# QCLovers/PyTDSCF

Measured on AMD Instinct MI355X. Metric: tdvp_sweeps_per_sec, higher is better.
Workload: dtype c128; 1 GPU; C4: synthetic exciton chain L=64 d=16 D=1024 M=32; L=64, d=16, D=1024, M=32, integrator=lanczos, steps_per_half_sweep=8, parallelism=single, approximate=False

## Files before the change

### pytdscf_amd/csrc/engine.h

```cpp
#pragma once
#include <functional>
#include <map>
#include <memory>
#include <string>
#include <vector>

#include "../../include/mitdvp.h"
#include "common.h"
#include "krylov_dev.h"
#include "qr.h"
#include "small_site.h"
#include "svd.h"
#include "vecops.h"

namespace mitdvp {

struct DevBuf {
  zc* p = nullptr;
  size_t n = 0;
  DevBuf() = default;
  DevBuf(const DevBuf&) = delete;
  DevBuf& operator=(const DevBuf&) = delete;
  DevBuf(DevBuf&& o) noexcept : p(o.p), n(o.n) { o.p = nullptr; o.n = 0; }
  DevBuf& operator=(DevBuf&& o) noexcept {
    if (this != &o) { release(); p = o.p; n = o.n; o.p = nullptr; o.n = 0; }
    return *this;
  }
  ~DevBuf() { release(); }
  void release() {
    if (p) (void)hipFree(p);
    p = nullptr;
    n = 0;
  }
  void reserve(size_t elems) {
    if (elems <= n) return;
    release();
    if (elems == 0) return;
    HIP_CHECK(hipMalloc(&p, elems * sizeof(zc)));
    n = elems;
  }
  void grow_preserve(size_t elems, size_t used, hipStream_t st) {
    if (elems <= n) return;
    zc* q = nullptr;
    HIP_CHECK(hipMalloc(&q, elems * sizeof(zc)));
    if (p && used) {
      HIP_CHECK(hipMemcpyAsync(q, p, used * sizeof(zc), hipMemcpyDeviceToDevice, st));
      HIP_CHECK(hipStreamSynchronize(st));
    }
    release();
    p = q;
    n = elems;
  }
};

struct ApplyPlan {
  bool trim_l = false, trim_r = false, edge = false, fold_l = false, fold_r = false;
  int strassen_l = 0, strassen_r = 0;
};

struct MpoSite {
  int ml = 0, d = 0, mr = 0;
  DevBuf w2l;
  DevBuf w2r;
  DevBuf w2lt, w2rt, kl_l, kl_r;
  int kl_stride_l = 0, kl_stride_r = 0;
  double sp_frac_l = 1.0, sp_frac_r = 1.0;
  struct SpSeg { int r0, r1; bool dense; int tile0; };
  std::vector<SpSeg> seg_l, seg_r;
  DevBuf w2el;
  DevBuf w2er;
  std::vector<hzc> whost;
  std::vector<char> nzblk;
  struct EnvFold {
    std::vector<int> t0; DevBuf ws, wg; bool reuse = false; hzc reuse_alpha; DevBuf ws_reuse;
    DevBuf ws_list, ws_reuse_list, wg_list; size_t wg_list_stride = 0;
  };
  struct EdgeCache {
    bool valid = false;
    unsigned long long s = 0, e = 0;
    std::vector<hzc> lam, mu;
    bool has_l = false, has_r = false;
    int skip = 0;
    DevBuf w_l, w_r;
    DevBuf w_l_list, w_r_list;
    DevBuf w_lf, w_rf;
    bool lf_ok = false, rf_ok = false;
    EnvFold envf[2];
    void rebuild(hipStream_t st, const MpoSite& w, unsigned long long S, unsigned long long E, const std::vector<hzc>& lam,
                 const std::vector<hzc>& mu);
  };
  mutable EdgeCache edge;
  DevBuf wtr;
  int ntr = 0, mltr = 0, mrtr = 0;
  int dtr = 0;
  bool set = false;
};
struct Operator {
  std::vector<MpoSite> sites;
  hzc shift{0.0, 0.0};
};

typedef int (*CollFn)(void* user, int op, void* dev_ptr, size_t nbytes);
enum { COLL_ALLGATHER = 0, COLL_ALLREDUCE = 1 };

struct PhaseTimer {
  hipEvent_t a, b;
  int kind;
  bool closed;
};

class SiteShard;
class Batch;
void cu_range_claim(int device, int first, int count);
void cu_range_release(int device, int first, int count);
int cu_ranges_claimed(int device);

class Engine {
  friend class SiteShard;
  friend class Batch;
// ... 108 lines not shown
  void copy_out(double* dst, const zc* src, size_t elems);
  void fold_block(int op_id, bool conj_bra, bool from_left, const double* in, int d, int m, double* out, int first = 0,
                  int count = -1);
  void site_rdm_blocks(int isite, const double* TL, const double* TR, double* out);
  hipStream_t stream() const { return st_; }
  int kprev_get(int p);
  void kprev_set(int p, int k);
  void set_small_kernels(bool on);
  void check_device_errors() { ss_check(); }
  const SmallSync::Last& small_last() const { return ss_.last; }
  const MpoSite& mpo(int op_id, int isite);
  mitdvp_config cfg;

 private:
  int ptr_mode_ = 0;
  struct CuClaim {
    int dev = -1, first = 0, count = 0;
    ~CuClaim() { if (dev >= 0) cu_range_release(dev, first, count); }
  } cu_claim_;
  bool qr_gauge_free_ = true;
  bool trim_identity_ = true;
  int edge_mode_ = -1;
  int fold_mode_ = -1;
  int strassen_mode_ = -1;
  bool strassen_batched_ = true;
  bool strassen_fuse_ = true;
  DevBuf str_l_, str_r_, str_v_, str_m_;
  static bool try_reserve(DevBuf& b, size_t elems);
  void strassen_side(const zc* fixed, bool fixed_is_a, const zc* psi, long ldpsi, zc* out, long hm, long hn, long hk, bool accumulate,
                     int level);
  int fold_env_mode_ = -1;
  bool env_reuse_ = true;
  bool core_lists_ = true;
  struct EnvChecked { const MpoSite* w = nullptr; const zc* blk[2] = {nullptr, nullptr}; int n[2] = {0, 0}; int lvl[2] = {0, 0}; } env_chk_;
  EnvChecked take_env_checked() { const EnvChecked c = env_chk_; env_chk_ = EnvChecked{}; return c; }
  struct IdentRecord { double dev[128]; hzc lam[128]; };
  static_assert(sizeof(IdentRecord) == 128 * 8 + 128 * 16 && sizeof(IdentRecord) <= 4 * NPART * sizeof(zc), "layout of the identity-check record");
  const IdentRecord& identity_sets(const zc* L, int ml, int dl, unsigned long long ms, const zc* R, int mr, int dr, unsigned long long me);
  void identity_blocks(const zc* L, int dl, int ml, const zc* R, int dr, int mr, bool* left, bool* right);
  int L_;
  hipStream_t st_ = nullptr;
  std::vector<int> dl_, dd_, dr_, gauge_;
  std::vector<DevBuf> site_;
  std::vector<std::vector<int>> sub_;
  std::vector<int> subn_;
  std::map<int, Operator> ops_;
  int center_ = -1;
  bool segment_ = false;
  int bnd_dl_ = 1, bnd_ml_ = 1, bnd_dr_ = 1, bnd_mr_ = 1;
  int bond_ = -1, bond_dim_ = 0, bond_site_ = 0;

  std::vector<DevBuf> envL_, envR_;
  std::vector<char> envL_ok_, envR_ok_;
  std::vector<DevBuf> pool_;
  size_t pool_cap_ = 48;
  DevBuf pool_get(size_t elems);
  void pool_put(DevBuf&& b);

  DevBuf X_, Y_, V_, Vdiag_, tmp1_, tmp2_, sig_, sig2_, qrwork_, red_;
  int max_diag_krylov_ = 64;
  MappedHost<zc> h_red_;
  MappedHost<unsigned> h_seq_;
  unsigned seq_tag_ = 0;
  KryDev* kst_ = nullptr;
  MappedHost<KryPub> h_kpub_;
  unsigned kry_tag_ = 0;
// ... 98 lines not shown
```

### pytdscf_amd/csrc/engine.hip

```cpp
#include "engine_internal.h"
#include "engine_krylov.inc"
#include "rccl_dyn.h"

namespace mitdvp {

Engine::Engine(const mitdvp_config& c) : cfg(c), L_(c.nsite) {
  if (c.nsite < 1) throw ArgError("nsite must be >= 1");
  if (c.max_krylov < 1 || c.max_krylov > MAXK - 1) throw ArgError("max_krylov must be in [1, 20]");
  if (c.integrator != MITDVP_LANCZOS && c.integrator != MITDVP_ARNOLDI) throw ArgError("bad integrator");
  if (c.relax < 0 || c.relax > 2) throw ArgError("relax must be 0, 1 or 2");
  max_diag_krylov_ = c.max_diag_krylov > 0 ? c.max_diag_krylov : 64;
  if (const char* e = std::getenv("MITDVP_SMALL_KERNELS")) small_kernels_ = std::atoi(e) != 0;
  if (const char* e = std::getenv("MITDVP_SPARSE_W")) sparse_w_ = std::atoi(e) != 0;
  if (const char* e = std::getenv("MITDVP_TRIM_IDENTITY")) trim_identity_ = std::atoi(e) != 0;
  if (const char* e = std::getenv("MITDVP_EDGE_APPLY")) edge_mode_ = std::atoi(e);
  if (const char* e = std::getenv("MITDVP_FOLD_APPLY")) fold_mode_ = std::atoi(e);
  if (const char* e = std::getenv("MITDVP_FOLD_STRASSEN")) strassen_mode_ = std::atoi(e);
  if (const char* e = std::getenv("MITDVP_STRASSEN_BATCH")) strassen_batched_ = std::atoi(e) != 0;
  if (const char* e = std::getenv("MITDVP_STRASSEN_FUSE")) strassen_fuse_ = std::atoi(e) != 0;
  if (const char* e = std::getenv("MITDVP_FOLD_ENV")) fold_env_mode_ = std::atoi(e);
  if (const char* e = std::getenv("MITDVP_FOLD_ENV_REUSE")) env_reuse_ = std::atoi(e) != 0;
  if (const char* e = std::getenv("MITDVP_CORE_LISTS")) core_lists_ = std::atoi(e) != 0;
  if (const char* e = std::getenv("MITDVP_QR_GAUGE_FREE")) qr_gauge_free_ = std::atoi(e) != 0;
  if (const char* e = std::getenv("MITDVP_KEFF_IDENT")) keff_ident_ = std::atoi(e) != 0;
  int ndev = 0;
  HIP_CHECK(hipGetDeviceCount(&ndev));
  if (ndev < 1) throw HipError("no HIP device visible: the MI355X engine has no CPU fallback");
  if (c.device < 0 || c.device >= ndev) throw ArgError("bad device ordinal");
  HIP_CHECK(hipSetDevice(c.device));
  HIP_CHECK(hipDeviceGetAttribute(&n_cu_, hipDeviceAttributeMultiprocessorCount, c.device));
  if (c.cu_count > 0) {
    if (c.cu_first < 0 || c.cu_first + c.cu_count > n_cu_ || c.cu_count % 8 != 0 || c.cu_first % 8 != 0)
      throw ArgError("cu_first / cu_count: a multiple of 8 compute units inside the device (8 k units = k CUs on every XCD)");
    std::vector<uint32_t> mask((size_t)(n_cu_ + 31) / 32, 0u);
    for (int u = c.cu_first; u < c.cu_first + c.cu_count; ++u) mask[(size_t)u / 32] |= 1u << (u % 32);
    cu_range_claim(c.device, c.cu_first, c.cu_count);
    cu_claim_.dev = c.device; cu_claim_.first = c.cu_first; cu_claim_.count = c.cu_count;
    HIP_CHECK(hipExtStreamCreateWithCUMask(&st_, (uint32_t)mask.size(), mask.data()));
    n_cu_ = c.cu_count;
    ss_.max_grid = c.cu_count;
    ss_.partitioned = true;
  } else {
    HIP_CHECK(hipStreamCreate(&st_));
  }
  qr_hist_ = qr_history_new();
  dl_.assign(L_, 0); dd_.assign(L_, 0); dr_.assign(L_, 0); gauge_.assign(L_, -1);
  site_.resize(L_);
  sub_.assign(L_, {}); subn_.assign(L_, 0);
  envL_.resize(L_ + 1); envR_.resize(L_ + 1);
  envL_ok_.assign(L_ + 1, 0); envR_ok_.assign(L_ + 1, 0);
  kprev_.assign(L_, 0);
  red_.reserve(RED_TOTAL);
  red_elems_ = RED_TOTAL;
  h_red_.alloc(RED_TOTAL * sizeof(zc));
  h_seq_.alloc(64);
// ... 702 lines not shown
```

### pytdscf_amd/csrc/engine_apply.hip

```cpp
#include "engine_internal.h"
#include "core_lists.h"

namespace mitdvp {

constexpr long STRASSEN_MIN_TILES = 256;

double Engine::w_stage(const MpoSite* sp, int side, const zc* w2, int d, int mout, int min_, int ncol, int nbatch) {
  ZgemmDesc g = zgemm_desc(w2, X_.p, Y_.p, d * mout, ncol, min_ * d);
  g.batch = nbatch; g.strideA = 0; g.strideB = (long)min_ * d * ncol; g.strideC = (long)d * mout * ncol;
  const bool use = sp && sparse_w_ && ncol >= 64 && (side == 0 ? sp->kl_l.p : sp->kl_r.p) &&
                   (side == 0 ? sp->sp_frac_l : sp->sp_frac_r) <= 0.6;
  if (!use) {
    zgemm(st_, g);
    return 1.0;
  }
  const zc* wt = side == 0 ? sp->w2lt.p : sp->w2rt.p;
  const int* kl = reinterpret_cast<const int*>(side == 0 ? sp->kl_l.p : sp->kl_r.p);
  const int stride = side == 0 ? sp->kl_stride_l : sp->kl_stride_r;
  const auto& segs = side == 0 ? sp->seg_l : sp->seg_r;
  const int K = min_ * d;
  for (int pass = 0; pass < 2; ++pass)
    for (const auto& sgm : segs) {
      if (sgm.dense != (pass == 0)) continue;
      ZgemmDesc h = g;
      h.A = wt + (size_t)sgm.r0 * K;
      h.M = sgm.r1 - sgm.r0;
      h.rowmap_p = d; h.rowmap_s1 = (long)mout * ncol; h.rowmap_s2 = ncol; h.rowmap_r0 = sgm.r0;
      if (!sgm.dense) { h.klist = kl + (size_t)sgm.tile0 * stride; h.klist_stride = stride; }
      h.tile_cfg = (sgm.dense && h.M <= 32) ? 2 : 1;
      zgemm(st_, h);
      cnt_.n_launch += 1;
    }
  cnt_.n_launch -= 1;
  return side == 0 ? sp->sp_frac_l : sp->sp_frac_r;
// ... 213 lines not shown
  if (same) return;
  const hzc* W = w.whost.data();
  std::vector<hzc> wl((size_t)d * ml * d, hzc(0, 0)), wr((size_t)d * d * mr, hzc(0, 0));
  valid = has_l = has_r = false;
  for (int c = 0; c < ml; ++c)
    for (int t = 0; t < mr; ++t) {
      if (!w.nzblk[(size_t)c * mr + t]) continue;
      const bool in_s = (S >> c) & 1ull;
      const hzc f = in_s ? lam[c] : mu[t];
      if (f == hzc(0.0, 0.0)) continue;
      for (int i = 0; i < d; ++i)
        for (int j = 0; j < d; ++j) {
          const hzc v = f * W[(((size_t)c * d + i) * d + j) * mr + t];
          if (in_s) wr[(size_t)i * d * mr + (size_t)j * mr + t] += v;
          else wl[(size_t)i * ml * d + (size_t)c * d + j] += v;
        }
      (in_s ? has_r : has_l) = true;
    }
  w_l.reserve(wl.size());
  w_r.reserve(wr.size());
  HIP_CHECK(hipMemcpyAsync(w_l.p, wl.data(), wl.size() * sizeof(zc), hipMemcpyHostToDevice, st));
  HIP_CHECK(hipMemcpyAsync(w_r.p, wr.data(), wr.size() * sizeof(zc), hipMemcpyHostToDevice, st));
  auto upload_list = [&](DevBuf& b, const std::vector<unsigned char>& blob, size_t at = 0) {
    HIP_CHECK(hipMemcpyAsync(reinterpret_cast<unsigned char*>(b.p) + at, blob.data(), blob.size(), hipMemcpyHostToDevice, st));
    HIP_CHECK(hipStreamSynchronize(st));
  };
  {
    const std::vector<unsigned char> ll = build_fold_list(wl.data(), d, ml, (long)ml * d, 1, d);
    const std::vector<unsigned char> lr = build_fold_list(wr.data(), d, mr, (long)d * mr, mr, 1);
    w_l_list.reserve(ll.size() / sizeof(zc));
    w_r_list.reserve(lr.size() / sizeof(zc));
    upload_list(w_l_list, ll);
    upload_list(w_r_list, lr);
  }
  w_lf.reserve(wl.size());
  w_rf.reserve(wr.size());
  lf_ok = zgemm_reduce_pack_core(st, w_l.p, (long)ml * d, d, ml * d, w_lf.p);
  rf_ok = zgemm_reduce_pack_core(st, w_r.p, (long)d * mr, d, d * mr, w_rf.p);
  for (int side = 0; side < 2; ++side) {
    const int mi = side == 0 ? ml : mr, mo = side == 0 ? mr : ml;
    const unsigned long long I = side == 0 ? S : E;
    const std::vector<hzc>& wt = side == 0 ? lam : mu;
    auto blk = [&](int in, int out) { return side == 0 ? (size_t)in * mr + out : (size_t)out * mr + in; };
    auto Wel = [&](int in, int i, int j, int out) {
      return side == 0 ? W[(((size_t)in * d + i) * d + j) * mr + out] : W[(((size_t)out * d + i) * d + j) * mr + in];
    };
    EnvFold& f = envf[side];
    f.t0.clear();
    for (int out = 0; out < mo; ++out)
      for (int in = 0; in < mi; ++in)
        if (!((I >> in) & 1ull) && w.nzblk[blk(in, out)]) { f.t0.push_back(out); break; }
    std::vector<hzc> ws((size_t)d * d * mo, hzc(0, 0)), wg(std::max<size_t>(f.t0.size(), 1) * d * mi * d, hzc(0, 0));
    for (int in = 0; in < mi; ++in) {
      if (!((I >> in) & 1ull)) continue;
      for (int out = 0; out < mo; ++out) {
        if (!w.nzblk[blk(in, out)]) continue;
        for (int i = 0; i < d; ++i)
          for (int j = 0; j < d; ++j) ws[((size_t)i * d + j) * mo + out] += wt[in] * Wel(in, i, j, out);
      }
    }
    for (size_t k = 0; k < f.t0.size(); ++k)
      for (int in = 0; in < mi; ++in) {
        if (((I >> in) & 1ull) || !w.nzblk[blk(in, f.t0[k])]) continue;
        for (int i = 0; i < d; ++i)
          for (int j = 0; j < d; ++j) wg[((k * d + i) * mi + in) * d + j] = Wel(in, i, j, f.t0[k]);
      }
// ... 56 lines not shown
  const bool skip = edge_cand && w.edge.skip > 0;
  if (skip) w.edge.skip -= 1;
  if (!edge_cand || skip) {
    identity_blocks(trim_identity_ && dl >= 256 && ml > 1 ? Lb : nullptr, dl, ml,
                    trim_identity_ && dr >= 256 && mr > 1 ? Rb : nullptr, dr, mr, &plan.trim_l, &plan.trim_r);
    return plan;
  }
  unsigned long long S = 0, E = 0;
  std::vector<hzc> lam(ml), mu(mr);
  for (int attempt = (w.edge.valid ? 0 : 1); attempt < 2; ++attempt) {
    const unsigned long long ms = attempt == 0 ? w.edge.s : ~0ull, me = attempt == 0 ? w.edge.e : ~0ull;
    const IdentRecord& h = identity_sets(Lb, ml, dl, ms, Rb, mr, dr, me);
    S = E = 0;
    for (int c = 0; c < ml; ++c) { lam[c] = h.lam[c]; if (((ms >> c) & 1ull) && h.dev[c] < 1e-13) S |= 1ull << c; }
    for (int t = 0; t < mr; ++t) { mu[t] = h.lam[64 + t]; if (((me >> t) & 1ull) && h.dev[64 + t] < 1e-13) E |= 1ull << t; }
    if (attempt == 0 && (S != w.edge.s || E != w.edge.e)) continue;
    break;
  }
  plan.trim_l = ml > 1 && (S & 1ull) && std::abs(lam[0] - 1.0) < 1e-13;
  plan.trim_r = mr > 1 && ((E >> (mr - 1)) & 1ull) && std::abs(mu[mr - 1] - 1.0) < 1e-13;
  for (int c = 0; c < ml; ++c)
    for (int t = 0; t < mr; ++t)
      if (w.nzblk[(size_t)c * mr + t] && !((S >> c) & 1ull) && !((E >> t) & 1ull)) {
        w.edge.skip = 16;
        return plan;
      }
  w.edge.rebuild(st_, w, S, E, lam, mu);
  plan.edge = true;
  env_chk_ = EnvChecked{&w, {Lb, Rb}, {dl, dr}};
  plan.fold_r = w.edge.has_r && can_fold_r;
  plan.fold_l = w.edge.has_l && can_fold_l;
  if (plan.fold_r || plan.fold_l) {
    timer_begin(11);
    if (plan.fold_r)
      fold_env_core(st_, Rb, w.edge.w_r.p, Y_.p, dr, mr, d, (long)d * mr, mr, 1, (long)dr * d * dr, (long)d * dr, dr, 1,
                    core_lists_ ? w.edge.w_r_list.p : nullptr);
    if (plan.fold_l)
      fold_env_core(st_, Lb, w.edge.w_l.p, X_.p, dl, ml, d, (long)ml * d, 1, d, (long)dl * d, (long)d * dl * d, 1, d,
                    core_lists_ ? w.edge.w_l_list.p : nullptr);
    const size_t quarter = (size_t)dl * d * dr / 4;
    auto tiles_fill = [](long pm, long pn) { return ((pm + 63) / 64) * ((pn + 63) / 64) >= STRASSEN_MIN_TILES; };
    auto level_of = [&](long rows, long cols, long klen) {
      if (strassen_mode_ == 0 || rows % 2 || cols % 2 || klen % 2) return 0;
      const bool four = rows % 4 == 0 && cols % 4 == 0 && klen % 4 == 0;
      if (strassen_mode_ > 0) return strassen_mode_ >= 2 && four ? 2 : 1;
      if (four && tiles_fill(rows / 4, cols / 4)) return 2;
      return tiles_fill(rows / 2, cols / 2) ? 1 : 0;
    };
    auto pack = [&](const zc* op, long n, DevBuf& f, int which, int want) {
      const long h = n / 2, q = n / 4;
      const size_t two = (strassen_fuse_ && which == STRASSEN_A ? 0 : 7 * quarter) + 49 * (quarter / 4);
      if (want == 2 && try_reserve(f, 49 * (size_t)q * q) && try_reserve(str_v_, two) && try_reserve(str_m_, two)) {
        strassen_operands2(st_, op, n, q, q, f.p, which);
        cnt_.n_launch += 1;
        return 2;
      }
      if (want == 0 || !try_reserve(f, 7 * (size_t)h * h) || !try_reserve(str_v_, 7 * quarter) || !try_reserve(str_m_, 7 * quarter))
        return 0;
      strassen_operands(st_, op, n, h, h, f.p, which);
      cnt_.n_launch += 1;
      return 1;
    };
    if (plan.fold_r) plan.strassen_r = pack(Y_.p, (long)d * dr, str_r_, STRASSEN_BT, level_of(dl, (long)d * dr, (long)d * dr));
    if (plan.fold_l) plan.strassen_l = pack(X_.p, (long)dl * d, str_l_, STRASSEN_A, level_of((long)dl * d, dr, (long)dl * d));
    env_chk_.lvl[0] = plan.strassen_l;
    env_chk_.lvl[1] = plan.strassen_r;
    timer_end();
    cnt_.n_launch += (plan.fold_r ? 1 : 0) + (plan.fold_l ? 1 : 0);
    if (std::getenv("MITDVP_EDGE_TRACE"))
      fprintf(stderr, "[mitdvp] folded sides of a site: R %s, L %s\n",
              plan.strassen_r == 2 ? "49 quarter-size products" : plan.strassen_r ? "seven half-size products" : plan.fold_r ? "plain product" : "not folded",
              plan.strassen_l == 2 ? "49 quarter-size products" : plan.strassen_l ? "seven half-size products" : plan.fold_l ? "plain product" : "not folded");
  }
  return plan;
}

void Engine::heff_apply(const zc* L, const MpoSite& w, const zc* R, const zc* psi, zc* out, int dl, int d, int dr,
                        hzc shift, const ApplyPlan& plan) {
  SmallChain sc;
  if (small_ok() && chain_heff(sc, L, w, R, dl, d, dr, false)) {
    timer_begin(10);
    small_apply(st_, ss_, sc, psi, out, ss_partials(sc), make_double2(shift.real(), shift.imag()), shift != hzc(0.0, 0.0));
    timer_end();
    cnt_.n_launch += 1;
    cnt_.n_heff += 1;
    cnt_.heff_flops += 8.0 * ((double)dl * dl * w.ml * d * dr + (double)dl * dr * w.ml * w.mr * d * d + (double)dl * dr * dr * w.mr * d);
    return;
  }
  if (plan.edge) heff_apply_edge(L, w, R, psi, out, dl, d, dr, plan);
  else heff_apply_rect(L, w, R, psi, out, dl, dl, d, dr, dr, plan);
  if (shift != hzc(0.0, 0.0))
    vec_axpby(st_, out, psi, (long)dl * d * dr, make_double2(shift.real(), shift.imag()), make_double2(1.0, 0.0));
}

void Engine::keff_apply_rect(const zc* L, const zc* R, const zc* sig, zc* out, int dlo, int dli, int dro, int dri,
                             int m) {
  int a0, a1;
  const bool sharded = shard_range(dlo, a0, a1);
  const int na = a1 - a0;
  timer_begin(2);
  {
    ZgemmDesc g = zgemm_desc(L + (size_t)a0 * m * dli, sig, X_.p, na * m, dri, dli);
    zgemm(st_, g);
  }
  {
// ... 219 lines not shown
```

### pytdscf_amd/csrc/engine_segment.hip

```cpp
#include "engine_internal.h"
#include "engine_krylov.inc"

namespace mitdvp {

void Engine::replace_site(int i, const double* reim, int gauge) {
  if (i < 0 || i >= L_ || !site_[i].p) throw ArgError("replace_site: bad or unset site");
  const size_t e = (size_t)dl_[i] * dd_[i] * dr_[i];
  copy_in(site_[i].p, reim, e);
  gauge_[i] = gauge;
  if (gauge == MITDVP_GAUGE_PSI) center_ = i;
  else if (center_ == i) center_ = -1;
}

void Engine::reshape_site(int i, const double* reim, int l, int n, int r, int gauge) {
  if (i < 0 || i >= L_ || !site_[i].p) throw ArgError("reshape_site: bad or unset site");
  if (l < 1 || r < 1 || n != dd_[i]) throw ArgError("reshape_site: bad shape");
  if (i != 0 && i != L_ - 1) throw ArgError("reshape_site: only a block's first or last site faces a junction");
  if ((i > 0 && l != dl_[i]) || (i < L_ - 1 && r != dr_[i])) throw ArgError("reshape_site: only the outer bond may change");
  const size_t e = (size_t)l * n * r;
  site_[i].reserve(e);
  copy_in(site_[i].p, reim, e);
  dl_[i] = l; dr_[i] = r; gauge_[i] = gauge;
  if (gauge == MITDVP_GAUGE_PSI) center_ = i;
  else if (center_ == i) center_ = -1;
// ... 40 lines not shown

void Engine::site_exp(double dt) {
  require_ready();
  if (center_ < 0) throw ArgError("site_exp: no centre site");
  const int p = center_;
  if (!envL_ok_[p] || !envR_ok_[p + 1]) throw ArgError("site_exp: the environment blocks around the centre are not built");
  local_site_exp(p, dt);
  ss_check();
}

void Engine::heff_apply_center(const double* in, double* out, int* flags) {
  require_ready();
  if (center_ < 0) throw ArgError("heff_apply_center: no centre site");
  const int p = center_;
  if (!envL_ok_[p] || !envR_ok_[p + 1]) throw ArgError("heff_apply_center: the environment blocks around the centre are not built");
  const MpoSite& w = mpo(0, p);
  if (dd_[p] != w.d) throw ArgError("MPO physical dimension differs from the site tensor's");
  const int dl = dl_[p], d = dd_[p], dr = dr_[p];
  const size_t n = (size_t)dl * d * dr;
  const zc* Lb = envL_[p].p;
  const zc* Rb = envR_[p + 1].p;
  DevBuf x = pool_get(n), y = pool_get(n);
  if (in) copy_in(x.p, in, n);
  else HIP_CHECK(hipMemcpyAsync(x.p, site_[p].p, n * sizeof(zc), hipMemcpyDeviceToDevice, st_));
  const ApplyPlan plan = choose_apply_forms(Lb, w, Rb, dl, d, dr);
  SmallChain sc;
  const bool small = small_ok() && chain_heff(sc, Lb, w, Rb, dl, d, dr, false);
  const bool edge = plan.edge && !small;
  const bool sparse = !small && !edge && sparse_w_ && dr >= 64 && w.kl_l.p && w.sp_frac_l <= 0.6;
  if (flags)
    *flags = (plan.trim_l && !small && !edge ? 1 : 0) | (plan.trim_r && !small && !edge ? 2 : 0) | (sparse ? 4 : 0) | (small ? 8 : 0) |
             (edge ? 16 : 0) | (edge && plan.fold_r ? 0x20 : 0) | (edge && plan.fold_l ? 0x40 : 0) |
             (edge && plan.strassen_r ? 0x80 : 0) | (edge && plan.strassen_l ? 0x100 : 0) |
             (edge && plan.strassen_r == 2 ? 0x200 : 0) | (edge && plan.strassen_l == 2 ? 0x400 : 0);
  heff_apply(Lb, w, Rb, x.p, y.p, dl, d, dr, op(0).shift, plan);
  copy_out(out, y.p, n);
  pool_put(std::move(x)); pool_put(std::move(y));
}

void Engine::split_center(bool forward) {
  require_ready();
  if (center_ < 0) throw ArgError("split_center: no centre site");
  const int p = center_;
  const MpoSite& w = mpo(0, p);
  const int dl = dl_[p], d = dd_[p], dr = dr_[p];
  DevBuf spare = pool_get(V_.n / MAXK);
  if (forward) {
    if (!envL_ok_[p]) throw ArgError("split_center: left environment missing");
    timer_begin(3);
    long nl = 0;
    qr_thin(st_, site_[p].p, dl * d, dr, spare.p, sig_.p, qrwork_.p, &nl, qr_hist_, qr_gauge_free_);
    timer_end();
    cnt_.n_launch += nl; cnt_.n_qr += 1;
    std::swap(site_[p], spare);
    gauge_[p] = MITDVP_GAUGE_A;
    pool_put(std::move(envL_[p + 1]));
    envL_[p + 1] = pool_get((size_t)dr * w.mr * dr);
    env_update(envL_[p].p, site_[p].p, w.w2l.p, envL_[p + 1].p, dl, w.ml, d, dr, w.mr, w.w2el.p, &w, 0);
    envL_ok_[p + 1] = 1;
    bond_ = p + 1; bond_dim_ = dr;
  } else {
    if (!envR_ok_[p + 1]) throw ArgError("split_center: right environment missing");
    gauge_qr_right(site_[p].p, dl, d, dr, spare.p, tmp2_.p, sig_.p);
    std::swap(site_[p], spare);
    gauge_[p] = MITDVP_GAUGE_B;
    pool_put(std::move(envR_[p]));
    envR_[p] = pool_get((size_t)dl * w.ml * dl);
// ... 171 lines not shown
```

### pytdscf_amd/csrc/vecops.h

```cpp
#pragma once
#include "common.h"
#include "small_chain_plan.h"

namespace mitdvp {

constexpr int NPART = 256;

constexpr int SMALL_VEC_EPT = 16;
constexpr long SMALL_VEC_N = 1024L * SMALL_VEC_EPT;

struct Coefs {
  zc c[MAXK];
};

int vec_blocks(long n);
void vec_dot(hipStream_t st, const zc* x, const zc* y, long n, bool conj_x, zc* out_p );
void vec_sumsq(hipStream_t st, const zc* x, long n, double* out_p );
void vec_lanczos_update(hipStream_t st, zc* v, const zc* vm1, const zc* vm2 , long n,
                        const zc* alpha_p, const double* betaprev_p, double* out_p);
void vec_lanczos_update_deferred(hipStream_t st, zc* v, const zc* ul, const zc* ulm1 , long n, const zc* alpha_raw_p,
                                 const double* nrm_all, int l, bool orthodox, double eps, double* out_p);
void vec_lanczos_step_small(hipStream_t st, zc* w, const zc* x, const zc* vl, const zc* vm2 , long n,
                            zc* alpha_p, const double* betaprev_p, double* nrm_p, double eps);
void vec_scale_inv_norm(hipStream_t st, zc* v, long n, const double* nrm_p, double eps);
void vec_multi_dot(hipStream_t st, const zc* V, long ldv, int k, const zc* v, long n, zc* out_p );
void vec_arnoldi_update(hipStream_t st, zc* v, const zc* V, long ldv, int k, long n, const zc* h_p, double* out_p);
void vec_lincomb(hipStream_t st, zc* out , const zc* V, long ldv, int k, const Coefs& c, long n,
                 double* nrm_p );
void vec_axpby(hipStream_t st, zc* y, const zc* x, long n, zc a, zc b);
void vec_scale(hipStream_t st, zc* y, long n, zc a);
void vec_randn(hipStream_t st, zc* out, long n, uint64_t seed);
void set_identity(hipStream_t st, zc* out, int rows, int cols, long ld);
void vec_copy_raw(hipStream_t st, zc* dst, const zc* src, size_t n);
void ident_deviation(hipStream_t st, const zc* blk, long ld, int n, double* out_dev);
void ident_deviation_multi(hipStream_t st, const zc* base, int nblk, long blk_stride, long ld, int n, double* out_dev,
                           zc* lam_dev, unsigned long long mask = ~0ull, bool clear = true);
void fold_env_core(hipStream_t st, const zc* env, const zc* w, zc* G, int n, int m, int d, long wi, long wj, long wm, long gi,
                   long gp, long gj, long gq, const void* list = nullptr);
void gram_env_core(hipStream_t st, const zc* G, const zc* ws, zc* out, int n, int m, int d, const void* list = nullptr);
void gram_mirror_lower(hipStream_t st, zc* G, int n, int d);
enum { STRASSEN_A = 0, STRASSEN_B = 1, STRASSEN_BT = 2 };
void strassen_operands(hipStream_t st, const zc* src, long ld, long hr, long hc, zc* dst, int which, int batch = 1,
                       long sstride = 0, long dstride = 0);
void strassen_operands2(hipStream_t st, const zc* src, long ld, long qr, long qc, zc* dst, int which);
void strassen_combine(hipStream_t st, const zc* M, long hr, long hc, zc* out, long ldo, bool accumulate, int batch = 1,
                      long mstride = 0, long ostride = 0);
void strassen_combine2(hipStream_t st, const zc* M, long qr, long qc, zc* out, long ldo, bool accumulate);
void copy2d(hipStream_t st, zc* dst, long ldd, const zc* src, long lds, long rows, int cols, int zero_to, zc a,
            bool accumulate);
struct BlockList { int n; int idx[64]; zc f[64]; };
void gather_blocks(hipStream_t st, zc* dst, int n_dst, const zc* src, int m_src, long rows, int cols, const BlockList& bl);
void fill_scaled_blocks(hipStream_t st, zc* X, long ldx, int pos0, const zc* sig, long rows, int cols, const BlockList& bl);
void accum_scaled_blocks(hipStream_t st, zc* out, const zc* X, long ldx, const zc* sig, long rows, int cols, const BlockList& bl,
                         zc both);
void col_sumsq(hipStream_t st, const zc* x, long rows, int cols, double* out );
void row_sumsq(hipStream_t st, const zc* x, int rows, long cols, double* out );
void shell_sumsq(hipStream_t st, const zc* x, int n, double* out );
void transpose_batched(hipStream_t st, const zc* in, zc* out, int rows, int cols, long ldi, long ldo, int batch,
                       long in_bs, long out_bs);
void phys_diag(hipStream_t st, const zc* C, zc* out, int dl, int n, int dr, bool trace);
void permute_0213(hipStream_t st, const zc* in, zc* out, long n0, int n1, int n2, int n3);
void clock_probe(hipStream_t st, long iters, double* host_out3 );
void where_probe(const uint32_t* mask, int nwords, int nblocks, size_t lds_bytes, int spin_us, int* host_out);
void permute5(hipStream_t st, const zc* in, zc* out, const int dims[5], const long in_strides[5], const int* map2);
void scale_cols(hipStream_t st, zc* x, long rows, int cols, long ld, const double* sc_dev);
void transpose_rev3(hipStream_t st, const zc* in, zc* out, int na, int nj, int ns);

}
```

### pytdscf_amd/csrc/vecops.hip

```cpp
#include "vecops.h"
#include "core_lists.h"
#include "krylov_dev.h"

#include <algorithm>

namespace mitdvp {

__device__ __forceinline__ double wave_sum(double v) {
#pragma unroll
  for (int o = 32; o > 0; o >>= 1) v += __shfl_down(v, o, 64);
  return v;
}

__device__ __forceinline__ double block_sum(double v, double* sh ) {
  v = wave_sum(v);
  const int lane = threadIdx.x & 63, w = threadIdx.x >> 6;
  __syncthreads();
  if (lane == 0) sh[w] = v;
  __syncthreads();
  if (threadIdx.x == 0) sh[4] = sh[0] + sh[1] + sh[2] + sh[3];
  __syncthreads();
  return sh[4];
}

__device__ __forceinline__ zc sum_partials_z(const zc* p, int np, double* sh) {
  double re = 0, im = 0;
  for (int i = threadIdx.x; i < np; i += 256) { re += p[i].x; im += p[i].y; }
  re = block_sum(re, sh);
  im = block_sum(im, sh);
  return make_double2(re, im);
}
__device__ __forceinline__ double sum_partials_d(const double* p, int np, double* sh) {
  double re = 0;
  for (int i = threadIdx.x; i < np; i += 256) re += p[i];
// ... 990 lines not shown
    }
  }
}
__global__ __launch_bounds__(256) void k_gram_mirror_lower(zc* G, int n, int d) {
  __shared__ zc tile[32][33];
  int i = 1, j = blockIdx.z;
  while (j >= i) { j -= i; ++i; }
  const long ldg = (long)d * n;
  const int q0 = blockIdx.x * 32, p0 = blockIdx.y * 32;
  const int tx = threadIdx.x & 31, ty = threadIdx.x >> 5;
  const zc* src = G + ((long)j * n) * ldg + (long)i * n;
  zc* dst = G + ((long)i * n) * ldg + (long)j * n;
  for (int r = ty; r < 32; r += 8) {
    const int q = q0 + r, p = p0 + tx;
    if (q < n && p < n) tile[r][tx] = src[(long)q * ldg + p];
  }
  __syncthreads();
  for (int r = ty; r < 32; r += 8) {
    const int p = p0 + r, q = q0 + tx;
    if (p < n && q < n) {
      const zc v = tile[tx][r];
      dst[(long)p * ldg + q] = make_double2(v.x, -v.y);
    }
  }
}
void gram_mirror_lower(hipStream_t st, zc* G, int n, int d) {
  if (n < 1 || d < 2) return;
  if (n > 65535 || d > 64) throw ArgError("gram_mirror_lower: d <= 64 and bond dimension <= 65535");
  const int nt = (n + 31) / 32;
  hipLaunchKernelGGL(k_gram_mirror_lower, dim3(nt, nt, d * (d - 1) / 2), dim3(256), 0, st, G, n, d);
  HIP_CHECK(hipGetLastError());
}

struct StrassenTab { int q1[7], q2[7], sg[7]; };
constexpr StrassenTab kStrassenTabs[3] = {
    {{0, 2, 0, 3, 0, 2, 1}, {3, 3, 0, 0, 1, 0, 3}, {1, 1, 0, 0, 1, -1, -1}},
    {{0, 0, 1, 2, 3, 0, 2}, {3, 0, 3, 0, 0, 1, 3}, {1, 0, -1, -1, 0, 1, 1}},
    {{0, 0, 2, 1, 3, 0, 1}, {3, 0, 3, 0, 0, 2, 3}, {1, 0, -1, -1, 0, 1, 1}}};
template <int W>
__global__ __launch_bounds__(256) void k_strassen_operands(const zc* __restrict__ src, long ld, long hr, long hc,
                                                           zc* __restrict__ dst, long sstride, long dstride) {
  constexpr StrassenTab t = kStrassenTabs[W];
  const long c = (long)blockIdx.x * 256 + threadIdx.x;
  if (c >= hc) return;
  const long blk = hr * hc;
  src += blockIdx.z * sstride;
  dst += blockIdx.z * dstride;
  for (long r = blockIdx.y; r < hr; r += gridDim.y) {
    zc q[4];
    q[0] = src[r * ld + c];
    q[1] = src[r * ld + hc + c];
    q[2] = src[(hr + r) * ld + c];
    q[3] = src[(hr + r) * ld + hc + c];
#pragma unroll
    for (int k = 0; k < 7; ++k) {
      const zc a = q[t.q1[k]], b = q[t.q2[k]];
      zc o = a;
      if (t.sg[k] > 0) { o.x += b.x; o.y += b.y; }
      if (t.sg[k] < 0) { o.x -= b.x; o.y -= b.y; }
      dst[k * blk + r * hc + c] = o;
    }
  }
}
template <int W>
__global__ __launch_bounds__(256) void k_strassen_operands2(const zc* __restrict__ src, long ld, long qr, long qc,
                                                            zc* __restrict__ dst) {
  constexpr StrassenTab t = kStrassenTabs[W];
  const long c = (long)blockIdx.x * 256 + threadIdx.x;
  if (c >= qc) return;
  const long blk = qr * qc;
  for (long r = blockIdx.y; r < qr; r += gridDim.y) {
// ... 151 lines not shown
```

Measured before the change: 0.04565 sweeps/s.

## Build Strassen operand factors directly from environment and MPO core in one MFMA kernel

New measurement: 0.04597 sweeps/s (median of 6 runs). Within noise of the previous version (+0.7%).

```diff
diff --git a/pytdscf_amd/csrc/engine.h b/pytdscf_amd/csrc/engine.h
--- a/pytdscf_amd/csrc/engine.h
+++ b/pytdscf_amd/csrc/engine.h
@@ -56,6 +56,7 @@
 struct ApplyPlan {
   bool trim_l = false, trim_r = false, edge = false, fold_l = false, fold_r = false;
   int strassen_l = 0, strassen_r = 0;
+  bool direct_l = false, direct_r = false;
 };
 
 struct MpoSite {
@@ -83,8 +84,10 @@
     int skip = 0;
     DevBuf w_l, w_r;
     DevBuf w_l_list, w_r_list;
+    DevBuf w_rd[2];
     DevBuf w_lf, w_rf;
     bool lf_ok = false, rf_ok = false;
+    bool rd_ok[2] = {false, false};
     EnvFold envf[2];
     void rebuild(hipStream_t st, const MpoSite& w, unsigned long long S, unsigned long long E, const std::vector<hzc>& lam,
                  const std::vector<hzc>& mu);
@@ -259,6 +262,7 @@
   int fold_env_mode_ = -1;
   bool env_reuse_ = true;
   bool core_lists_ = true;
+  int fold_direct_mode_ = -1;
   struct EnvChecked { const MpoSite* w = nullptr; const zc* blk[2] = {nullptr, nullptr}; int n[2] = {0, 0}; int lvl[2] = {0, 0}; } env_chk_;
   EnvChecked take_env_checked() { const EnvChecked c = env_chk_; env_chk_ = EnvChecked{}; return c; }
   struct IdentRecord { double dev[128]; hzc lam[128]; };
diff --git a/pytdscf_amd/csrc/engine.hip b/pytdscf_amd/csrc/engine.hip
--- a/pytdscf_amd/csrc/engine.hip
+++ b/pytdscf_amd/csrc/engine.hip
@@ -21,6 +21,7 @@
   if (const char* e = std::getenv("MITDVP_FOLD_ENV")) fold_env_mode_ = std::atoi(e);
   if (const char* e = std::getenv("MITDVP_FOLD_ENV_REUSE")) env_reuse_ = std::atoi(e) != 0;
   if (const char* e = std::getenv("MITDVP_CORE_LISTS")) core_lists_ = std::atoi(e) != 0;
+  if (const char* e = std::getenv("MITDVP_FOLD_DIRECT")) fold_direct_mode_ = std::atoi(e);
   if (const char* e = std::getenv("MITDVP_QR_GAUGE_FREE")) qr_gauge_free_ = std::atoi(e) != 0;
   if (const char* e = std::getenv("MITDVP_KEFF_IDENT")) keff_ident_ = std::atoi(e) != 0;
   int ndev = 0;
diff --git a/pytdscf_amd/csrc/engine_apply.hip b/pytdscf_amd/csrc/engine_apply.hip
--- a/pytdscf_amd/csrc/engine_apply.hip
+++ b/pytdscf_amd/csrc/engine_apply.hip
@@ -1,5 +1,6 @@
 #include "engine_internal.h"
 #include "core_lists.h"
+#include "fold_direct.h"
 
 namespace mitdvp {
 
@@ -279,6 +280,14 @@
     w_r_list.reserve(lr.size() / sizeof(zc));
     upload_list(w_l_list, ll);
     upload_list(w_r_list, lr);
+  }
+  for (int lv = 1; lv <= 2; ++lv) {
+    rd_ok[lv - 1] = has_r && d % fold_direct_parts(lv) == 0;
+    if (!rd_ok[lv - 1]) continue;
+    const std::vector<hzc> wc = build_fold_direct_cores(wr.data(), d, mr, lv);
+    w_rd[lv - 1].reserve(wc.size());
+    HIP_CHECK(hipMemcpyAsync(w_rd[lv - 1].p, wc.data(), wc.size() * sizeof(zc), hipMemcpyHostToDevice, st));
+    HIP_CHECK(hipStreamSynchronize(st));
   }
   w_lf.reserve(wl.size());
   w_rf.reserve(wr.size());
@@ -401,12 +410,6 @@
   plan.fold_l = w.edge.has_l && can_fold_l;
   if (plan.fold_r || plan.fold_l) {
     timer_begin(11);
-    if (plan.fold_r)
-      fold_env_core(st_, Rb, w.edge.w_r.p, Y_.p, dr, mr, d, (long)d * mr, mr, 1, (long)dr * d * dr, (long)d * dr, dr, 1,
-                    core_lists_ ? w.edge.w_r_list.p : nullptr);
-    if (plan.fold_l)
-      fold_env_core(st_, Lb, w.edge.w_l.p, X_.p, dl, ml, d, (long)ml * d, 1, d, (long)dl * d, (long)d * dl * d, 1, d,
-                    core_lists_ ? w.edge.w_l_list.p : nullptr);
     const size_t quarter = (size_t)dl * d * dr / 4;
     auto tiles_fill = [](long pm, long pn) { return ((pm + 63) / 64) * ((pn + 63) / 64) >= STRASSEN_MIN_TILES; };
     auto level_of = [&](long rows, long cols, long klen) {
@@ -416,30 +419,67 @@
       if (four && tiles_fill(rows / 4, cols / 4)) return 2;
       return tiles_fill(rows / 2, cols / 2) ? 1 : 0;
     };
-    auto pack = [&](const zc* op, long n, DevBuf& f, int which, int want) {
+    auto reserve = [&](long n, DevBuf& f, int which, int want) {
       const long h = n / 2, q = n / 4;
       const size_t two = (strassen_fuse_ && which == STRASSEN_A ? 0 : 7 * quarter) + 49 * (quarter / 4);
-      if (want == 2 && try_reserve(f, 49 * (size_t)q * q) && try_reserve(str_v_, two) && try_reserve(str_m_, two)) {
-        strassen_operands2(st_, op, n, q, q, f.p, which);
-        cnt_.n_launch += 1;
-        return 2;
-      }
+      if (want == 2 && try_reserve(f, 49 * (size_t)q * q) && try_reserve(str_v_, two) && try_reserve(str_m_, two)) return 2;
       if (want == 0 || !try_reserve(f, 7 * (size_t)h * h) || !try_reserve(str_v_, 7 * quarter) || !try_reserve(str_m_, 7 * quarter))
         return 0;
-      strassen_operands(st_, op, n, h, h, f.p, which);
-      cnt_.n_launch += 1;
       return 1;
     };
-    if (plan.fold_r) plan.strassen_r = pack(Y_.p, (long)d * dr, str_r_, STRASSEN_BT, level_of(dl, (long)d * dr, (long)d * dr));
-    if (plan.fold_l) plan.strassen_l = pack(X_.p, (long)dl * d, str_l_, STRASSEN_A, level_of((long)dl * d, dr, (long)dl * d));
+    auto pack = [&](const zc* op, long n, DevBuf& f, int which, int lv) {
+      if (lv == 2) strassen_operands2(st_, op, n, n / 4, n / 4, f.p, which);
+      else if (lv == 1) strassen_operands(st_, op, n, n / 2, n / 2, f.p, which);
+      cnt_.n_launch += lv ? 1 : 0;
+    };
+    auto direct_wanted = [&](int side, int m, int lv) {
+      return lv >= 1 && fold_direct_mode_ != 0 && fold_direct_ok(side, dl, d, dr, m, lv) &&
+             (fold_direct_mode_ > 0 || fold_direct_rule(side, d, lv));
+    };
+    if (plan.fold_r) {
+      const long n = (long)d * dr;
+      const int lv = reserve(n, str_r_, STRASSEN_BT, level_of(dl, n, n));
+      plan.strassen_r = lv;
+      plan.direct_r = direct_wanted(1, mr, lv) && w.edge.rd_ok[lv - 1];
+      if (plan.direct_r) {
+        const int e = d / fold_direct_parts(lv);
+        const long q = (long)e * dr;
+        fold_direct(st_, Rb, 0, 1, w.edge.w_rd[lv - 1].p, (long)e * e * mr, fold_direct_factors(lv), str_r_.p, q * q, dr, mr, e, e,
+                    (long)e * mr, mr, 1, (long)dr * q, q, dr, 1, true);
+      } else {
+        fold_env_core(st_, Rb, w.edge.w_r.p, Y_.p, dr, mr, d, (long)d * mr, mr, 1, (long)dr * d * dr, (long)d * dr, dr, 1,
+                      core_lists_ ? w.edge.w_r_list.p : nullptr);
+        pack(Y_.p, n, str_r_, STRASSEN_BT, lv);
+      }
+      cnt_.n_launch += 1;
+    }
+    if (plan.fold_l) {
+      const long n = (long)dl * d;
+      const int lv = reserve(n, str_l_, STRASSEN_A, level_of(n, dr, n));
+      plan.strassen_l = lv;
+      const int nf = fold_direct_factors(lv), e = lv ? dl / fold_direct_parts(lv) : dl;
+      plan.direct_l = direct_wanted(0, ml, lv) && (size_t)nf * e * ml * e <= X_.n;
+      if (plan.direct_l) {
+        const long q = (long)e * d;
+        fold_direct_pack(st_, Lb, e, ml, lv, X_.p);
+        fold_direct(st_, X_.p, (long)e * ml * e, nf, w.edge.w_l.p, 0, 1, str_l_.p, q * q, e, ml, d, d, (long)ml * d, 1, d, q,
+                    (long)d * q, 1, d, false);
+        cnt_.n_launch += 1;
+      } else {
+        fold_env_core(st_, Lb, w.edge.w_l.p, X_.p, dl, ml, d, (long)ml * d, 1, d, (long)dl * d, (long)d * dl * d, 1, d,
+                      core_lists_ ? w.edge.w_l_list.p : nullptr);
+        pack(X_.p, n, str_l_, STRASSEN_A, lv);
+      }
+      cnt_.n_launch += 1;
+    }
     env_chk_.lvl[0] = plan.strassen_l;
     env_chk_.lvl[1] = plan.strassen_r;
     timer_end();
-    cnt_.n_launch += (plan.fold_r ? 1 : 0) + (plan.fold_l ? 1 : 0);
     if (std::getenv("MITDVP_EDGE_TRACE"))
-      fprintf(stderr, "[mitdvp] folded sides of a site: R %s, L %s\n",
+      fprintf(stderr, "[mitdvp] folded sides of a site: R %s, L %s; factors built directly: %s\n",
               plan.strassen_r == 2 ? "49 quarter-size products" : plan.strassen_r ? "seven half-size products" : plan.fold_r ? "plain product" : "not folded",
-              plan.strassen_l == 2 ? "49 quarter-size products" : plan.strassen_l ? "seven half-size products" : plan.fold_l ? "plain product" : "not folded");
+              plan.strassen_l == 2 ? "49 quarter-size products" : plan.strassen_l ? "seven half-size products" : plan.fold_l ? "plain product" : "not folded",
+              plan.direct_r && plan.direct_l ? "R, L" : plan.direct_r ? "R" : plan.direct_l ? "L" : "none");
   }
   return plan;
 }
diff --git a/pytdscf_amd/csrc/engine_segment.hip b/pytdscf_amd/csrc/engine_segment.hip
--- a/pytdscf_amd/csrc/engine_segment.hip
+++ b/pytdscf_amd/csrc/engine_segment.hip
@@ -96,7 +96,8 @@
     *flags = (plan.trim_l && !small && !edge ? 1 : 0) | (plan.trim_r && !small && !edge ? 2 : 0) | (sparse ? 4 : 0) | (small ? 8 : 0) |
              (edge ? 16 : 0) | (edge && plan.fold_r ? 0x20 : 0) | (edge && plan.fold_l ? 0x40 : 0) |
              (edge && plan.strassen_r ? 0x80 : 0) | (edge && plan.strassen_l ? 0x100 : 0) |
-             (edge && plan.strassen_r == 2 ? 0x200 : 0) | (edge && plan.strassen_l == 2 ? 0x400 : 0);
+             (edge && plan.strassen_r == 2 ? 0x200 : 0) | (edge && plan.strassen_l == 2 ? 0x400 : 0) |
+             (edge && plan.direct_r ? 0x800 : 0) | (edge && plan.direct_l ? 0x1000 : 0);
   heff_apply(Lb, w, Rb, x.p, y.p, dl, d, dr, op(0).shift, plan);
   copy_out(out, y.p, n);
   pool_put(std::move(x)); pool_put(std::move(y));
diff --git a/pytdscf_amd/csrc/fold_direct.h b/pytdscf_amd/csrc/fold_direct.h
--- /dev/null
+++ b/pytdscf_amd/csrc/fold_direct.h
@@ -0,0 +1,76 @@
+#pragma once
+#include <complex>
+#include <cstddef>
+#include <vector>
+
+namespace mitdvp {
+
+struct StrassenTab { int q1[7], q2[7], sg[7]; };
+constexpr StrassenTab kStrassenTabs[3] = {
+    {{0, 2, 0, 3, 0, 2, 1}, {3, 3, 0, 0, 1, 0, 3}, {1, 1, 0, 0, 1, -1, -1}},
+    {{0, 0, 1, 2, 3, 0, 2}, {3, 0, 3, 0, 0, 1, 3}, {1, 0, -1, -1, 0, 1, 1}},
+    {{0, 0, 2, 1, 3, 0, 1}, {3, 0, 3, 0, 0, 2, 3}, {1, 0, -1, -1, 0, 1, 1}}};
+
+struct FoldDirectTerms { int n; int sg[4], U[4], V[4]; };
+constexpr int fold_direct_parts(int level) { return 1 << level; }
+constexpr int fold_direct_factors(int level) { return level == 2 ? 49 : 7; }
+constexpr FoldDirectTerms fold_direct_terms(int which, int level, int k) {
+  const StrassenTab t = kStrassenTabs[which];
+  FoldDirectTerms f = {0, {0, 0, 0, 0}, {0, 0, 0, 0}, {0, 0, 0, 0}};
+  if (level == 1) {
+    for (int g = 0; g < 2; ++g) {
+      if (g == 1 && t.sg[k] == 0) continue;
+      const int Q = g ? t.q2[k] : t.q1[k];
+      f.sg[f.n] = g ? t.sg[k] : 1; f.U[f.n] = Q >> 1; f.V[f.n] = Q & 1;
+      ++f.n;
+    }
+    return f;
+  }
+  const int k1 = k / 7, k2 = k % 7;
+  for (int h = 0; h < 2; ++h) {
+    if (h == 1 && t.sg[k2] == 0) continue;
+    const int P = h ? t.q2[k2] : t.q1[k2];
+    for (int g = 0; g < 2; ++g) {
+      if (g == 1 && t.sg[k1] == 0) continue;
+      const int Q = g ? t.q2[k1] : t.q1[k1];
+      f.sg[f.n] = (h ? t.sg[k2] : 1) * (g ? t.sg[k1] : 1);
+      f.U[f.n] = 2 * (Q >> 1) + (P >> 1);
+      f.V[f.n] = 2 * (Q & 1) + (P & 1);
+      ++f.n;
+    }
+  }
+  return f;
+}
+
+inline bool fold_direct_ok(int side, int dl, int d, int dr, int m, int level) {
+  if (level < 1 || level > 2 || m < 1 || m > 64 || d < 1 || dl < 1 || dr < 1) return false;
+  const int P = fold_direct_parts(level);
+  if (side == 1) return d % P == 0 && dr <= 65535;
+  return dl % P == 0 && dl / P <= 65535;
+}
+inline bool fold_direct_rule(int side, int d, int level) {
+  const int P = fold_direct_parts(level);
+  const int fill = side == 1 ? (d / P) * (d / P) : d;
+  return fill % 16 == 0 || fill % 16 >= 8;
+}
+
+inline std::vector<std::complex<double>> build_fold_direct_cores(const std::complex<double>* wr, int d, int m, int level) {
+  const int P = fold_direct_parts(level), nf = fold_direct_factors(level), e = d / P;
+  std::vector<std::complex<double>> out((size_t)nf * e * e * m, std::complex<double>(0.0, 0.0));
+  for (int k = 0; k < nf; ++k) {
+    const FoldDirectTerms f = fold_direct_terms(2, level, k);
+    for (int i = 0; i < e; ++i)
+      for (int j = 0; j < e; ++j)
+        for (int t = 0; t < m; ++t) {
+          std::complex<double> s(0.0, 0.0);
+          for (int u = 0; u < f.n; ++u) {
+            const std::complex<double> v = wr[((size_t)(e * f.U[u] + i) * d + (e * f.V[u] + j)) * m + t];
+            s = u == 0 ? v : f.sg[u] > 0 ? s + v : s - v;
+          }
+          out[(((size_t)k * e + i) * e + j) * m + t] = s;
+        }
+  }
+  return out;
+}
+
+}
diff --git a/pytdscf_amd/csrc/fold_direct.hip b/pytdscf_amd/csrc/fold_direct.hip
--- /dev/null
+++ b/pytdscf_amd/csrc/fold_direct.hip
@@ -0,0 +1,228 @@
+#include "vecops.h"
+#include "fold_direct.h"
+
+#include <algorithm>
+
+namespace mitdvp {
+
+typedef double fd4 __attribute__((ext_vector_type(4)));
+
+struct FoldDirectArgs {
+  const zc* env;
+  const zc* core;
+  zc* out;
+  long env_z, core_f, out_f, wi, wj, wm, gx, gp, gy, gq;
+  int n, m, dx, dy, nf_inner, cd_mode;
+};
+
+__device__ __forceinline__ int fd_cd_row(int mode, int lk, int r) { return mode == 0 ? lk + 4 * r : 4 * lk + r; }
+
+template <int KS>
+__device__ __forceinline__ void fd_load_core(const zc* __restrict__ cp, long wm, int m, int lk, double (&cr)[KS], double (&ci)[KS]) {
+#pragma unroll
+  for (int ks = 0; ks < KS; ++ks) {
+    const zc v = cp[min(4 * ks + lk, m - 1) * wm];
+    cr[ks] = v.x;
+    ci[ks] = v.y;
+  }
+}
+
+template <bool CORE_ROWS, bool M3, int KS>
+__global__ __launch_bounds__(256, (KS <= 8 ? 2 : 1)) void k_fold_direct(FoldDirectArgs a) {
+  constexpr int T = KS <= 8 ? 2 : 1;
+  const int lane = threadIdx.x & 63, li = lane & 15, lk = lane >> 4;
+  const int wave = __builtin_amdgcn_readfirstlane((int)(threadIdx.x >> 6));
+  const int p = blockIdx.y, z = blockIdx.z;
+  const int q0 = (blockIdx.x * 4 + wave) * (16 * T);
+  if (q0 >= a.n) return;
+  const zc* __restrict__ env = a.env + z * a.env_z + (long)p * a.m * a.n;
+  double er[T][KS], ei[T][KS];
+#pragma unroll
+  for (int t = 0; t < T; ++t)
+#pragma unroll
+    for (int ks = 0; ks < KS; ++ks) {
+      const int c = 4 * ks + lk, q = q0 + 16 * t + li;
+      const zc v = env[(long)min(c, a.m - 1) * a.n + min(q, a.n - 1)];
+      const bool in = c < a.m && q < a.n;
+      er[t][ks] = in ? v.x : 0.0;
+      ei[t][ks] = in ? v.y : 0.0;
+    }
+  const int ncore = a.dx * a.dy;
+  const int ngr = CORE_ROWS ? (ncore + 15) >> 4 : (a.dy + 15) >> 4;
+  const int nitems = (CORE_ROWS ? a.nf_inner : a.dx) * ngr;
+  auto core_of = [&](int it, const zc*& cp, bool& ok) {
+    const int o = it / ngr, g = it - o * ngr;
+    const int io = 16 * g + li;
+    if (CORE_ROWS) {
+      ok = io < ncore;
+      const int ic = ok ? io : 0, x = ic / a.dy, y = ic - x * a.dy;
+      cp = a.core + ((long)z * a.nf_inner + o) * a.core_f + x * a.wi + y * a.wj;
+    } else {
+      ok = io < a.dy;
+      cp = a.core + (long)z * a.nf_inner * a.core_f + o * a.wi + (ok ? io : 0) * a.wj;
+    }
+  };
+  double cr[KS], ci[KS], cs[KS], nr[KS], ni[KS];
+  bool nok;
+  auto take = [&]() {
+#pragma unroll
+    for (int ks = 0; ks < KS; ++ks) {
+      const bool in = nok && 4 * ks + lk < a.m;
+      cr[ks] = in ? nr[ks] : 0.0;
+      ci[ks] = in ? ni[ks] : 0.0;
+      cs[ks] = M3 ? cr[ks] + ci[ks] : -ci[ks];
+    }
+  };
+  {
+    const zc* cp;
+    core_of(0, cp, nok);
+    fd_load_core<KS>(cp, a.wm, a.m, lk, nr, ni);
+    take();
+  }
+  for (int it = 0; it < nitems; ++it) {
+    bool ok_next;
+    {
+      const zc* cp;
+      core_of(min(it + 1, nitems - 1), cp, ok_next);
+      fd_load_core<KS>(cp, a.wm, a.m, lk, nr, ni);
+    }
+    const int o = it / ngr, g = it - o * ngr;
+    long off[4];
+    bool okr[4];
+    const long base = ((long)z * a.nf_inner + (CORE_ROWS ? o : 0)) * a.out_f + p * a.gp;
+#pragma unroll
+    for (int r = 0; r < 4; ++r) {
+      const int row = fd_cd_row(a.cd_mode, lk, r);
+      if (CORE_ROWS) {
+        const int io = 16 * g + row, x = io / a.dy, y = io - x * a.dy;
+        okr[r] = io < ncore;
+        off[r] = base + x * a.gx + y * a.gy;
+      } else {
+        const int y = 16 * g + li;
+        okr[r] = y < a.dy;
+        off[r] = base + o * a.gx + y * a.gy;
+      }
+    }
+    const fd4 zero = {0.0, 0.0, 0.0, 0.0};
+    fd4 p1[T], p2[T], p3[T];
+#pragma unroll
+    for (int t = 0; t < T; ++t) {
+      p1[t] = zero; p2[t] = zero; p3[t] = zero;
+#pragma unroll
+      for (int ks = 0; ks < KS; ++ks) {
+        const double x = er[t][ks], y = ei[t][ks];
+        if (M3) {
+          double xo = x;
+          asm volatile("" : "+v"(xo));
+          const double s = xo + y;
+          p1[t] = CORE_ROWS ? __builtin_amdgcn_mfma_f64_16x16x4f64(cr[ks], x, p1[t], 0, 0, 0)
+                            : __builtin_amdgcn_mfma_f64_16x16x4f64(x, cr[ks], p1[t], 0, 0, 0);
+          p2[t] = CORE_ROWS ? __builtin_amdgcn_mfma_f64_16x16x4f64(ci[ks], y, p2[t], 0, 0, 0)
+                            : __builtin_amdgcn_mfma_f64_16x16x4f64(y, ci[ks], p2[t], 0, 0, 0);
+          p3[t] = CORE_ROWS ? __builtin_amdgcn_mfma_f64_16x16x4f64(cs[ks], s, p3[t], 0, 0, 0)
+                            : __builtin_amdgcn_mfma_f64_16x16x4f64(s, cs[ks], p3[t], 0, 0, 0);
+        } else {
+          p1[t] = CORE_ROWS ? __builtin_amdgcn_mfma_f64_16x16x4f64(cr[ks], x, p1[t], 0, 0, 0)
+                            : __builtin_amdgcn_mfma_f64_16x16x4f64(x, cr[ks], p1[t], 0, 0, 0);
+          p2[t] = CORE_ROWS ? __builtin_amdgcn_mfma_f64_16x16x4f64(cr[ks], y, p2[t], 0, 0, 0)
+                            : __builtin_amdgcn_mfma_f64_16x16x4f64(y, cr[ks], p2[t], 0, 0, 0);
+          p1[t] = CORE_ROWS ? __builtin_amdgcn_mfma_f64_16x16x4f64(cs[ks], y, p1[t], 0, 0, 0)
+                            : __builtin_amdgcn_mfma_f64_16x16x4f64(y, cs[ks], p1[t], 0, 0, 0);
+          p2[t] = CORE_ROWS ? __builtin_amdgcn_mfma_f64_16x16x4f64(ci[ks], x, p2[t], 0, 0, 0)
+                            : __builtin_amdgcn_mfma_f64_16x16x4f64(x, ci[ks], p2[t], 0, 0, 0);
+        }
+      }
+    }
+    __builtin_amdgcn_sched_barrier(0);
+    nok = ok_next;
+    take();
+#pragma unroll
+    for (int ks = 0; ks < KS; ++ks) asm volatile("" : "+v"(cr[ks]), "+v"(ci[ks]), "+v"(cs[ks]) : : "memory");
+    __builtin_amdgcn_sched_barrier(0);
+#pragma unroll
+    for (int t = 0; t < T; ++t) {
+      if (q0 + 16 * t >= a.n) continue;
+#pragma unroll
+      for (int r = 0; r < 4; ++r) {
+        const int q = q0 + 16 * t + (CORE_ROWS ? li : fd_cd_row(a.cd_mode, lk, r));
+        const double re = M3 ? p1[t][r] - p2[t][r] : p1[t][r], im = M3 ? p3[t][r] - p1[t][r] - p2[t][r] : p2[t][r];
+        if (okr[r] && q < a.n) a.out[off[r] + q * a.gq] = make_double2(re, im);
+      }
+    }
+  }
+}
+
+template <bool CORE_ROWS, bool M3>
+static void fold_direct_launch(hipStream_t st, const FoldDirectArgs& a, int nz) {
+  if (a.m <= 32) hipLaunchKernelGGL((k_fold_direct<CORE_ROWS, M3, 8>), dim3((a.n + 127) / 128, a.n, nz), dim3(256), 0, st, a);
+  else hipLaunchKernelGGL((k_fold_direct<CORE_ROWS, M3, 16>), dim3((a.n + 63) / 64, a.n, nz), dim3(256), 0, st, a);
+}
+
+void fold_direct(hipStream_t st, const zc* env, long env_z, int nz, const zc* core, long core_f, int nf_inner, zc* out, long out_f,
+                 int n, int m, int dx, int dy, long wi, long wj, long wm, long gx, long gp, long gy, long gq, bool core_rows,
+                 int mode3m) {
+  if (n < 1 || dx < 1 || dy < 1 || nz < 1 || nf_inner < 1) return;
+  if (m < 1 || m > 64 || n > 65535 || nz > 65535) throw ArgError("fold_direct: MPO bond in [1, 64], bond dimension and batch <= 65535");
+  FoldDirectArgs a;
+  a.env = env; a.core = core; a.out = out;
+  a.env_z = env_z; a.core_f = core_f; a.out_f = out_f;
+  a.wi = wi; a.wj = wj; a.wm = wm; a.gx = gx; a.gp = gp; a.gy = gy; a.gq = gq;
+  a.n = n; a.m = m; a.dx = dx; a.dy = dy; a.nf_inner = nf_inner;
+  a.cd_mode = zgemm_cd_mode(st);
+  const bool m3 = mode3m < 0 ? zgemm_default_mode() != 0 : mode3m != 0;
+  if (core_rows) { if (m3) fold_direct_launch<true, true>(st, a, nz); else fold_direct_launch<true, false>(st, a, nz); }
+  else { if (m3) fold_direct_launch<false, true>(st, a, nz); else fold_direct_launch<false, false>(st, a, nz); }
+  HIP_CHECK(hipGetLastError());
+}
+
+template <int LEVEL>
+struct FoldDirectTermTable { FoldDirectTerms f[fold_direct_factors(LEVEL)]; };
+template <int LEVEL>
+constexpr FoldDirectTermTable<LEVEL> fold_direct_term_table() {
+  FoldDirectTermTable<LEVEL> t = {};
+  for (int k = 0; k < fold_direct_factors(LEVEL); ++k) t.f[k] = fold_direct_terms(STRASSEN_A, LEVEL, k);
+  return t;
+}
+template <int LEVEL>
+__global__ __launch_bounds__(256) void k_fold_direct_pack(const zc* __restrict__ L, int e, int m, zc* __restrict__ dst) {
+  constexpr int P = fold_direct_parts(LEVEL), NF = fold_direct_factors(LEVEL);
+  constexpr FoldDirectTermTable<LEVEL> tab = fold_direct_term_table<LEVEL>();
+  const long col = (long)blockIdx.x * 256 + threadIdx.x;
+  const long me = (long)m * e;
+  if (col >= me) return;
+  const long c = col / e, b = col - c * e;
+  const long dl = (long)P * e, blk = (long)e * me;
+  for (long r = blockIdx.y; r < e; r += gridDim.y) {
+    zc s[P * P];
+#pragma unroll
+    for (int U = 0; U < P; ++U)
+#pragma unroll
+      for (int V = 0; V < P; ++V) s[P * U + V] = L[((U * e + r) * m + c) * dl + V * e + b];
+    zc* dp = dst + r * me + col;
+#pragma unroll
+    for (int k = 0; k < NF; ++k) {
+      zc o = s[P * tab.f[k].U[0] + tab.f[k].V[0]];
+#pragma unroll
+      for (int u = 1; u < 4; ++u) {
+        if (u >= tab.f[k].n) continue;
+        const zc v = s[P * tab.f[k].U[u] + tab.f[k].V[u]];
+        if (tab.f[k].sg[u] > 0) { o.x += v.x; o.y += v.y; }
+        else { o.x -= v.x; o.y -= v.y; }
+      }
+      *dp = o;
+      dp += blk;
+      asm volatile("" : "+v"(dp));
+    }
+  }
+}
+
+void fold_direct_pack(hipStream_t st, const zc* L, int e, int m, int level, zc* dst) {
+  if (e < 1 || m < 1) return;
+  if (level < 1 || level > 2) throw ArgError("fold_direct_pack: one or two levels");
+  const dim3 grid((unsigned)(((long)m * e + 255) / 256), (unsigned)std::min(e, 32768));
+  if (level == 2) hipLaunchKernelGGL(k_fold_direct_pack<2>, grid, dim3(256), 0, st, L, e, m, dst);
+  else hipLaunchKernelGGL(k_fold_direct_pack<1>, grid, dim3(256), 0, st, L, e, m, dst);
+  HIP_CHECK(hipGetLastError());
+}
+
+}
diff --git a/pytdscf_amd/csrc/vecops.h b/pytdscf_amd/csrc/vecops.h
--- a/pytdscf_amd/csrc/vecops.h
+++ b/pytdscf_amd/csrc/vecops.h
@@ -46,6 +46,10 @@
 void strassen_combine(hipStream_t st, const zc* M, long hr, long hc, zc* out, long ldo, bool accumulate, int batch = 1,
                       long mstride = 0, long ostride = 0);
 void strassen_combine2(hipStream_t st, const zc* M, long qr, long qc, zc* out, long ldo, bool accumulate);
+void fold_direct(hipStream_t st, const zc* env, long env_z, int nz, const zc* core, long core_f, int nf_inner, zc* out, long out_f,
+                 int n, int m, int dx, int dy, long wi, long wj, long wm, long gx, long gp, long gy, long gq, bool core_rows,
+                 int mode3m = -1);
+void fold_direct_pack(hipStream_t st, const zc* L, int e, int m, int level, zc* dst);
 void copy2d(hipStream_t st, zc* dst, long ldd, const zc* src, long lds, long rows, int cols, int zero_to, zc a,
             bool accumulate);
 struct BlockList { int n; int idx[64]; zc f[64]; };
diff --git a/pytdscf_amd/csrc/vecops.hip b/pytdscf_amd/csrc/vecops.hip
--- a/pytdscf_amd/csrc/vecops.hip
+++ b/pytdscf_amd/csrc/vecops.hip
@@ -1,5 +1,6 @@
 #include "vecops.h"
 #include "core_lists.h"
+#include "fold_direct.h"
 #include "krylov_dev.h"
 
 #include <algorithm>
@@ -1056,11 +1057,6 @@
   HIP_CHECK(hipGetLastError());
 }
 
-struct StrassenTab { int q1[7], q2[7], sg[7]; };
-constexpr StrassenTab kStrassenTabs[3] = {
-    {{0, 2, 0, 3, 0, 2, 1}, {3, 3, 0, 0, 1, 0, 3}, {1, 1, 0, 0, 1, -1, -1}},
-    {{0, 0, 1, 2, 3, 0, 2}, {3, 0, 3, 0, 0, 1, 3}, {1, 0, -1, -1, 0, 1, 1}},
-    {{0, 0, 2, 1, 3, 0, 1}, {3, 0, 3, 0, 0, 2, 3}, {1, 0, -1, -1, 0, 1, 1}}};
 template <int W>
 __global__ __launch_bounds__(256) void k_strassen_operands(const zc* __restrict__ src, long ld, long hr, long hc,
                                                            zc* __restrict__ dst, long sstride, long dstride) {
```
